# edlanglois/relearn

Measured on AMD Instinct MI355X. Metric: env-steps/sec (whole node), 64k-env CartPole TRPO, higher is better.
Workload: dtype f32; 1 GPU; CartPole(VisibleStepLimit 500) MLP-TRPO, 65536 envs total, T=128, policy 5-128-2, critic 5-128-1, CG 10, <=15 backtracks, 80 Adam critic steps per period; n_envs_total=65536, n_envs_per_gpu=65536, horizon=128, hidden=128, critic_steps=80, update_chains=policy and critic chains side by side on two streams, pipeline=none, parallelism=env-sharded x1 + no collective (one rank)

## Files before the change

include/relearn_hip.h:

```cpp
#ifndef RELEARN_HIP_H
#define RELEARN_HIP_H

#include <stddef.h>
#include <stdint.h>

#ifdef __cplusplus
extern "C" {
#endif

#define RL_ABI_VERSION 6

typedef enum {
  RL_OK = 0,
  RL_ERR_INVALID_ARGUMENT = 1,
  RL_ERR_HIP = 2,
  RL_ERR_NO_DEVICE = 3,
  RL_ERR_BUILD_AGENT = 4,
  RL_ERR_BUILD_ENV = 5,
  RL_ERR_BUFFER_FULL = 6,
  RL_ERR_PACKING = 7,
  RL_ERR_COMM = 8,
  RL_ERR_OPT_NAN = 9,
  RL_ERR_UNSUPPORTED = 10
} rl_status;
// ... 75 lines not shown
  uint64_t episodes_per_trial;
} rl_meta_bandit_config;
int32_t rl_meta_bandit_config_default(rl_meta_bandit_config *meta);
int32_t rl_env_create_meta_bandit(rl_engine *engine, const rl_env_config *cfg, const rl_meta_bandit_config *meta,
                                  rl_env **out);
int32_t rl_env_create_meta_bandit_wide(rl_engine *engine, const rl_env_config *cfg, const rl_meta_bandit_config *meta,
                                       rl_env **out);
int32_t rl_env_destroy(rl_env *env);
int32_t rl_env_dims(const rl_env *env, uint32_t *obs_dim, uint32_t *n_actions);
int32_t rl_env_reset(rl_env *env);
int32_t rl_env_observe(rl_env *env, float *obs_out);
int32_t rl_env_step(rl_env *env, const uint8_t *actions, float *reward_out, uint8_t *flag_out, float *obs_out,
                    float *term_obs_out);
int32_t rl_env_upload_actions(rl_env *env, const uint8_t *actions);
int32_t rl_env_step_resident(rl_env *env);
int32_t rl_env_get_state(rl_env *env, double *state4, int32_t *nv_pos, uint64_t *steps_remaining,
                         uint64_t *reset_count);
int32_t rl_env_set_state(rl_env *env, const double *state4, const int32_t *nv_pos, const uint64_t *steps_remaining,
                         const uint64_t *reset_count);

int32_t rl_debug_stream_words(rl_engine *engine, uint64_t seed, uint64_t stream, uint64_t first_word, uint32_t n_words,
                              uint32_t *words_out);
int32_t rl_debug_device_memory(uint64_t *live_bytes, uint64_t *live_allocations);

int32_t rl_mlp_create(rl_engine *engine, uint32_t in_dim, uint32_t hidden, uint32_t out_dim, rl_mlp **out);
typedef enum {
  RL_ACT_IDENTITY = 0,
  RL_ACT_RELU = 1,
  RL_ACT_SIGMOID = 2,
  RL_ACT_TANH = 3
} rl_activation;
int32_t rl_mlp_create_layers(rl_engine *engine, uint32_t in_dim, const uint32_t *hidden_sizes, uint32_t n_hidden,
                             uint32_t out_dim, int32_t activation, int32_t output_activation, rl_mlp **out);
int32_t rl_mlp_create_config(rl_engine *engine, uint32_t in_dim, const uint32_t *hidden_sizes, uint32_t n_hidden,
                             uint32_t out_dim, int32_t activation, int32_t output_activation, int32_t bias, rl_mlp **out);
int32_t rl_mlp_destroy(rl_mlp *mlp);
int32_t rl_mlp_num_params(const rl_mlp *mlp, uint64_t *n);
int32_t rl_mlp_init(rl_mlp *mlp, uint64_t seed);
typedef enum { RL_INIT_ZEROS = 0, RL_INIT_CONSTANT = 1, RL_INIT_UNIFORM = 2, RL_INIT_NORMAL = 3, RL_INIT_ORTHOGONAL = 4 } rl_init_kind;
typedef enum { RL_SCALE_CONSTANT = 0, RL_SCALE_FAN_IN = 1, RL_SCALE_FAN_OUT = 2, RL_SCALE_FAN_AVG = 3 } rl_variance_scale;
typedef struct {
  int32_t kind;
  int32_t scale;
  double value;
} rl_initializer;
int32_t rl_mlp_init_with(rl_mlp *mlp, uint64_t seed, const rl_initializer *kernel_init, const rl_initializer *bias_init);
// ... 264 lines not shown
```

relearn_amd/__init__.py:

```python
import atexit
import ctypes as C
import math
import os
import subprocess
import sys
import weakref

import numpy as np

_HERE = os.path.dirname(os.path.abspath(__file__))
LIB_PATH = os.environ.get("RELEARN_LIB", os.path.join(_HERE, "librelearn_hip.so"))
CSRC = os.path.join(_HERE, "csrc")

OK = 0
ERR_INVALID_ARGUMENT, ERR_HIP, ERR_NO_DEVICE, ERR_BUILD_AGENT, ERR_BUILD_ENV = 1, 2, 3, 4, 5
ERR_BUFFER_FULL, ERR_PACKING, ERR_COMM, ERR_OPT_NAN, ERR_UNSUPPORTED = 6, 7, 8, 9, 10
SUCC_CONTINUE, SUCC_TERMINATE, SUCC_INTERRUPT = 0, 1, 2
OPT_OK, OPT_LOSS_NOT_IMPROVING, OPT_CONSTRAINT_VIOLATED, OPT_NAN_LOSS, OPT_NAN_CONSTRAINT = range(5)
ENV_CARTPOLE, ENV_CHAIN, ENV_MEMORY, ENV_BANDIT, ENV_META_BANDIT = 0, 1, 2, 3, 4
BANDITS_UNIFORM_BERNOULLI, BANDITS_ONE_HOT, BANDITS_ROUND_ROBIN = 0, 1, 2
BANDIT_DISTRIBUTIONS = {"uniform_bernoulli": BANDITS_UNIFORM_BERNOULLI, "one_hot": BANDITS_ONE_HOT,
                        "round_robin": BANDITS_ROUND_ROBIN}
LIMIT_NONE, LIMIT_LATENT, LIMIT_VISIBLE = 0, 1, 2
BANDIT_AGENT_RANDOM, BANDIT_AGENT_TABULAR_Q, BANDIT_AGENT_UCB1 = 0, 1, 2
BANDIT_AGENT_THOMPSON = 4
BANDIT_AGENT_KINDS = {"random": BANDIT_AGENT_RANDOM, "tabular_q": BANDIT_AGENT_TABULAR_Q, "ucb1": BANDIT_AGENT_UCB1,
                      "thompson": BANDIT_AGENT_THOMPSON}
(BANDIT_STATE_ACTOR_POS, BANDIT_STATE_COUNTS, BANDIT_STATE_VALUES, BANDIT_STATE_VISITS,
 BANDIT_STATE_LN_TABLE, BANDIT_STATE_LOW_COUNTS, BANDIT_STATE_HIGH_COUNTS) = range(7)
(TRAJ_OBS, TRAJ_ACTION, TRAJ_REWARD, TRAJ_FLAG, TRAJ_TERM_OBS, TRAJ_VALUES, TRAJ_ADVANTAGES,
 TRAJ_RETURNS, TRAJ_TARGETS) = range(9)
VALUE_TARGET_REWARD_TO_GO, VALUE_TARGET_ONE_STEP_TD = 0, 1
OPTIMIZER_ADAM, OPTIMIZER_ADAMW, OPTIMIZER_SGD, OPTIMIZER_RMSPROP = 0, 1, 2, 3
KERNEL_CLASSES = ["env_step", "rollout", "values", "gae", "policy_pass", "backward", "reduce", "small",
                  "critic_fwd", "allreduce", "critic_fused", "policy_fused", "policy_fvp"]

ABI_SYMBOLS = [
    "rl_abi_version", "rl_debug_stream_words", "rl_debug_device_memory", "rl_device_count", "rl_engine_create", "rl_engine_destroy", "rl_engine_sync",
    "rl_last_error", "rl_engine_info", "rl_engine_set_kernel_variant", "rl_timer_begin", "rl_timer_end", "rl_profile_enable", "rl_profile_read",
    "rl_comm_available", "rl_comm_library_paths", "rl_comm_unique_id", "rl_comm_init", "rl_comm_destroy", "rl_comm_init_host",
    "rl_comm_ipc_handle", "rl_comm_init_ipc", "rl_comm_selftest",
    "rl_cartpole_params_default", "rl_env_create", "rl_env_create_bandit", "rl_meta_bandit_config_default", "rl_env_create_meta_bandit", "rl_env_create_meta_bandit_wide", "rl_env_destroy", "rl_env_dims", "rl_env_reset",
    "rl_env_observe", "rl_env_step", "rl_env_upload_actions", "rl_env_step_resident", "rl_env_get_state",
    "rl_env_set_state",
    "rl_mlp_create", "rl_mlp_create_layers", "rl_mlp_create_config", "rl_mlp_destroy", "rl_mlp_num_params", "rl_mlp_init", "rl_mlp_init_with", "rl_params_get", "rl_params_set",
    "rl_mlp_forward", "rl_gru_mlp_create", "rl_lstm_mlp_create", "rl_rnn_mlp_create", "rl_rnn_mlp_create_config", "rl_rnn_linear_create", "rl_rnn_chain_config_default", "rl_rnn_chain_create", "rl_rnn_chain_create_wide", "rl_rnn_mlp_init_with", "rl_seq_forward",
    "rl_traj_create", "rl_traj_destroy", "rl_traj_field_bytes", "rl_traj_read", "rl_traj_write",
    "rl_rollout", "rl_gae",
    "rl_trpo_config_default", "rl_trpo_update", "rl_policy_gradient", "rl_policy_fvp", "rl_policy_loss_kl",
    "rl_adam_config_default", "rl_adam_create", "rl_adam_destroy", "rl_adam_step_host",
    "rl_optimizer_config_default", "rl_optimizer_create", "rl_optimizer_step_host", "rl_optimizer_state_read",
    "rl_critic_update", "rl_critic_gradient", "rl_values_opt_config_default", "rl_values_opt_update",
    "rl_actor_critic_update", "rl_actor_critic_update_begin", "rl_actor_critic_update_finish", "rl_engine_set_serial_update",
    "rl_ppo_config_default", "rl_ppo_update", "rl_reinforce_update", "rl_reward_to_go",
    "rl_actor_to_cbor", "rl_module_from_cbor", "rl_tensor_def_to_cbor", "rl_tensor_def_from_cbor",
    "rl_indexed_type_space_to_cbor",
    "rl_dqn_config_default", "rl_dqn_create", "rl_dqn_create_recurrent", "rl_dqn_create_finite", "rl_dqn_destroy", "rl_dqn_exploration_rate",
    "rl_dqn_min_update_size", "rl_dqn_collect", "rl_dqn_update", "rl_dqn_replay_field_bytes", "rl_dqn_replay_read",
    "rl_dqn_minibatch_sample", "rl_dqn_minibatch_read", "rl_dqn_minibatch_gradient", "rl_dqn_agent_rng_pos",
    "rl_chain_tabular_q_train", "rl_chain_tabular_q_eval",
    "rl_summary_create", "rl_summary_destroy", "rl_summary_push", "rl_summary_push_dqn", "rl_summary_read",
# ... 670 lines not shown

    def close(self):
        if self.h:
            lib().rl_traj_destroy(self.h)
            self.h = C.c_void_p()

    def shape(self, field):
        n, T, D = self.n, self.T, self.D
        return {TRAJ_OBS: (D, T + 1, n), TRAJ_ACTION: (T, n), TRAJ_REWARD: (T, n), TRAJ_FLAG: (T, n),
                TRAJ_TERM_OBS: (D, T, n), TRAJ_VALUES: (T + 1, n), TRAJ_ADVANTAGES: (T, n),
                TRAJ_RETURNS: (T, n), TRAJ_TARGETS: (T, n)}[field]

    def read(self, field):
        out = np.zeros(self.shape(field), dtype=_TRAJ_DTYPES[field])
        _check(lib().rl_traj_read(self.h, C.c_int32(field), out.ctypes.data_as(C.c_void_p),
                                  C.c_uint64(out.nbytes)), self.eng.h)
        return out

    def write(self, field, arr):
        arr, ap = _ptr(arr, _TRAJ_DTYPES[field])
        assert arr.shape == self.shape(field), (arr.shape, self.shape(field))
        _check(lib().rl_traj_write(self.h, C.c_int32(field), ap, C.c_uint64(arr.nbytes)), self.eng.h)

    def read_all(self):
        return dict(obs=self.read(TRAJ_OBS), action=self.read(TRAJ_ACTION), reward=self.read(TRAJ_REWARD),
                    flag=self.read(TRAJ_FLAG), term_obs=self.read(TRAJ_TERM_OBS))

    def write_all(self, traj):
        self.write(TRAJ_OBS, traj["obs"])
        self.write(TRAJ_ACTION, traj["action"])
        self.write(TRAJ_REWARD, traj["reward"])
        self.write(TRAJ_FLAG, traj["flag"])
        self.write(TRAJ_TERM_OBS, traj["term_obs"])


def rollout(env, policy, traj):
    _check(lib().rl_rollout(env.h, policy.h, traj.h), env.eng.h)


def gae(traj, critic, gamma, lam):
    _check(lib().rl_gae(traj.h, critic.h, C.c_float(gamma), C.c_float(lam)), traj.eng.h)


def trpo_config_default():
    c = TrpoConfig()
    _check(lib().rl_trpo_config_default(C.byref(c)))
# ... 513 lines not shown
```

relearn_amd/csrc/abi.hip:

```cpp
#include <dlfcn.h>

#include <atomic>
#include <condition_variable>
#include <map>
#include <mutex>

#include "abi_internal.hpp"
#include "env_lanes.hpp"

thread_local std::string g_last_error_no_engine;

static std::atomic<uint64_t> g_device_bytes{0}, g_device_allocations{0};

void *rl_device_alloc(uint64_t bytes) {
  void *p = nullptr;
  RL_HIP_CHECK(hipMalloc(&p, bytes));
  g_device_bytes += bytes;
  g_device_allocations += 1;
  return p;
}

void rl_device_free(void *p, uint64_t bytes) {
  (void)hipFree(p);
  g_device_bytes -= bytes;
// ... 298 lines not shown
    if (compute_units) *compute_units = e->prop.multiProcessorCount;
  });
}

int32_t rl_timer_begin(rl_engine *e) {
  return guarded(e, [&] {
    RL_REQUIRE(e, "engine is NULL");
    RL_HIP_CHECK(hipEventRecord(e->ev_begin, e->stream));
  });
}

int32_t rl_timer_end(rl_engine *e, float *elapsed_ms) {
  return guarded(e, [&] {
    RL_REQUIRE(e && elapsed_ms, "NULL argument");
    RL_HIP_CHECK(hipEventRecord(e->ev_end, e->stream));
    RL_HIP_CHECK(hipEventSynchronize(e->ev_end));
    RL_HIP_CHECK(hipEventElapsedTime(elapsed_ms, e->ev_begin, e->ev_end));
  });
}

int32_t rl_engine_set_kernel_variant(rl_engine *e, int32_t variant) {
  return guarded(e, [&] {
    RL_REQUIRE(e, "engine is NULL");
    RL_REQUIRE(variant == 0 || variant == 1, "kernel variant must be 0 (best) or 1 (v1 reference kernels)");
    e->kernel_variant = variant;
  });
}

int32_t rl_engine_set_serial_update(rl_engine *e, int32_t serial) {
  return guarded(e, [&] {
    RL_REQUIRE(e, "engine is NULL");
    e->serial_update = serial != 0;
  });
}

int32_t rl_profile_enable(rl_engine *e, int32_t on) {
  return guarded(e, [&] {
    RL_REQUIRE(e, "engine is NULL");
    sync(e);
    prof_drain(e);
    e->profiling = on != 0;
  });
}

int32_t rl_profile_read(rl_engine *e, double *total_ms_out, uint64_t *launches_out, int32_t reset) {
  return guarded(e, [&] {
    RL_REQUIRE(e, "engine is NULL");
// ... 448 lines not shown

int32_t rl_debug_stream_words(rl_engine *engine, uint64_t seed, uint64_t stream, uint64_t first_word, uint32_t n_words,
                              uint32_t *words_out) {
  return guarded(engine, [&] {
    RL_REQUIRE(engine && words_out, "NULL argument");
    RL_REQUIRE(n_words > 0 && n_words <= (1u << 20), "n_words must be in [1, 2^20]");
    AgentKey key;
    rl_seed_from_u64(seed, key.w);
    DevMem tmp;
    uint32_t *d = tmp.alloc<uint32_t>(n_words);
    hipLaunchKernelGGL(k_debug_stream_words, dim3((n_words + 255) / 256), dim3(256), 0, engine->stream, key, stream,
                       first_word, n_words, d);
    RL_HIP_CHECK(hipGetLastError());
    d2h(engine, words_out, d, (size_t)n_words * sizeof(uint32_t));
  });
}

int32_t rl_debug_device_memory(uint64_t *live_bytes, uint64_t *live_allocations) {
  if (live_bytes) *live_bytes = g_device_bytes.load();
  if (live_allocations) *live_allocations = g_device_allocations.load();
  return RL_OK;
}

int32_t rl_env_upload_actions(rl_env *env, const uint8_t *actions) {
  return guarded(env ? env->eng : nullptr, [&] {
    RL_REQUIRE(env && actions, "NULL argument");
    check_actions(env, actions);
    h2d(env->eng, env->d_actions, actions, env->cfg.n_lanes);
  });
}

int32_t rl_env_step_resident(rl_env *env) {
  return guarded(env ? env->eng : nullptr, [&] {
    RL_REQUIRE(env, "env is NULL");
    launch_env_step(env);
    env->t_global += 1;
  });
}

int32_t rl_env_step(rl_env *env, const uint8_t *actions, float *reward_out, uint8_t *flag_out, float *obs_out,
                    float *term_obs_out) {
  return guarded(env ? env->eng : nullptr, [&] {
    RL_REQUIRE(env && actions, "NULL argument");
    check_actions(env, actions);
    rl_engine *e = env->eng;
    size_t n = env->cfg.n_lanes;
// ... 805 lines not shown
```

relearn_amd/csrc/abi_dqn.hip:

```cpp
#include "abi_internal.hpp"

extern "C" {

int32_t rl_dqn_config_default(rl_dqn_config *c) {
  return guarded(nullptr, [&] {
    RL_REQUIRE(c, "cfg is NULL");
    std::memset(c, 0, sizeof(*c));
    c->target = RL_DQN_TARGET_REWARD_TO_GO;
    c->exploration_kind = RL_SCHEDULE_LINEAR_ANNEALED;
    c->exploration_start = 1.0;
    c->exploration_end = 0.1;
    c->exploration_period = 10000000;
    c->minibatch_steps = 100000;
    c->opt_steps_per_update = 50;
    c->buffer_capacity = 0;
    c->episode_capacity = 0;
    c->update_kind = RL_COLLECT_FIRST_REST;
    c->update_first = 1000000;
    c->update_rest = 100000;
    c->discount_factor = 0.99f;
  });
}

static double dqn_exploration_rate(const rl_dqn *q, bool training) {
// ... 415 lines not shown
                         q->d_ep_off + o, q->d_counts + k, mb->d.obs, 0, mb->d.action, mb->d.adv, 0,
                         q->cfg.discount_factor, mb->d.flag);
    q->mem.ensure(q->d_q_next, (uint64_t)q->A * q->max_steps_mb);
    launch_gen_forward(mb, q->qnet, mb->d.obs + c.n_steps, (size_t)2 * c.n_steps, c.n_steps, q->d_q_next);
    launch_dqn_td_targets(q->eng, mb->d.adv, mb->d.flag, q->d_q_next, c.n_steps, q->A, q->cfg.discount_factor);
    return;
  }
  launch_dqn_build_minibatch(q->eng, q->rp, c.n_eps, q->d_ep_lane + o, q->d_ep_start + o, q->d_ep_len + o,
                             q->d_ep_off + o, mb->d.obs, (size_t)2 * c.n_steps, mb->d.action, mb->d.adv,
                             q->cfg.discount_factor, td ? 1 : 0, q->qnet);
}

static void dqn_sample_minibatch(rl_dqn *q, int sequential) {
  std::vector<DqnCountsDev> counts;
  std::vector<uint64_t> totals;
  dqn_draw_minibatches(q, sequential, 1, counts, totals);
  dqn_build_minibatch(q, 0, counts[0], totals[0]);
}

static void dqn_gradient(rl_dqn *q, rl_adam *step_opt = nullptr, int loss_slot = -1) {
  if (q->recurrent) return rdqn_gradient(q, step_opt, loss_slot);
  rl_traj *mb = q->mb;
  bool fused = false;
  if (q->eng->kernel_variant == 0)
    fused = q->td_in_kernel ? launch_dqn_step_bf16(mb, q->qnet, q->last_total_steps, q->cfg.discount_factor)
                            : launch_dqn_step_pair(mb, q->qnet, q->last_total_steps);
  PassRequest pass(RUN_DQN);
  pass.B_total = q->last_total_steps;
  pass.reduce = false;
  const SlabRows rows = fused ? SlabRows{mb->nbV2, mb->nbV2} : run_pass(q->qnet, mb, pass);
  if (step_opt && !q->eng->has_collective()) {
    launch_reduce_opt(mb, step_opt, rows.A, rows.B, loss_slot, q->last_total_steps);
    return;
  }
  const uint32_t P = (uint32_t)q->qnet->P;
  launch_reduce(mb, P, true, true, rows.A, rows.B);
  rl_allreduce_sum_f32(q->eng, mb->vec, P + 4);
  if (step_opt) launch_opt_step(mb, step_opt, loss_slot, q->last_total_steps);
}

static void rdqn_update(rl_dqn *q, rl_dqn_update_stats *stats, float *losses_out) {
  rl_engine *e = q->eng;
  if (e->n_ranks > 1)
    throw RlError(RL_ERR_UNSUPPORTED, "rl_dqn_update: an agent of rl_dqn_create_recurrent updates on one rank");
  q->global_steps = q->steps_per_lane * (uint64_t)q->rp.N;
  const uint64_t K = q->cfg.opt_steps_per_update;
  std::vector<DqnCountsDev> counts;
// ... 33 lines not shown
  }
  std::vector<float> h(K ? K : 1, 0.0f);
  if (K) d2h(e, h.data(), q->seq->losses, K * sizeof(float));
  if (losses_out && K) std::memcpy(losses_out, h.data(), K * sizeof(float));
  if (stats) {
    stats->opt_steps = K;
    stats->loss_first = K ? (double)h[0] : 0.0;
    stats->loss_last = K ? (double)h[K - 1] : 0.0;
    stats->global_steps = q->global_steps;
    stats->last_minibatch_steps = q->last_n_steps;
    stats->last_minibatch_episodes = q->last_n_eps;
  }
}

int32_t rl_dqn_update(rl_dqn *q, rl_dqn_update_stats *stats, float *losses_out) {
  return guarded(q ? q->eng : nullptr, [&] {
    RL_REQUIRE(q, "NULL argument");
    if (q->recurrent) return rdqn_update(q, stats, losses_out);
    rl_engine *e = q->eng;
    q->global_steps = q->steps_per_lane * (uint64_t)q->rp.N * (uint64_t)e->n_ranks;
    uint64_t K = q->cfg.opt_steps_per_update;
    const uint64_t D = q->rp.D, cap = q->max_steps_mb;
    const bool td = q->cfg.target == RL_DQN_TARGET_ONE_STEP_TD;
    const bool fused_shape = e->kernel_variant == 0 && fused_5_128_fits(q->mb, q->qnet, 2, false);
    const bool td_fused = td && fused_shape;
    const bool all_at_once = K > 1 && (!td || td_fused) && K * cap * (8 * D + 6) <= (8ull << 30);
    if (all_at_once) {
      q->mem.ensure(q->all_obs, K * D * 2 * cap);
      q->mem.ensure(q->all_target, K * cap);
      q->mem.ensure(q->all_action, K * cap);
      if (td) q->mem.ensure(q->all_flag, K * cap);
    }
    const bool pipelined = all_at_once && e->n_ranks == 1 && !e->profiling;
    std::vector<DqnCountsDev> counts;
    std::vector<uint64_t> totals;
    std::vector<uint32_t> chunk_end;
    if (pipelined) {
      for (uint64_t first = 0, size = 2; first < K; first += size, size *= 2) chunk_end.push_back((uint32_t)(first + size < K ? first + size : K));
      if (!q->draw_stream) RL_HIP_CHECK(hipStreamCreateWithFlags(&q->draw_stream, hipStreamNonBlocking));
      if (!q->main_event) RL_HIP_CHECK(hipEventCreateWithFlags(&q->main_event, hipEventDisableTiming));
      if (!q->h_counts) q->h_counts = q->mem.alloc_host<DqnCountsDev>(K, false);
      while (q->draw_events.size() < chunk_end.size()) {
        hipEvent_t ev;
        RL_HIP_CHECK(hipEventCreateWithFlags(&ev, hipEventDisableTiming));
        q->draw_events.push_back(ev);
      }
      RL_HIP_CHECK(hipEventRecord(q->main_event, e->stream));
// ... 216 lines not shown
```

relearn_amd/csrc/abi_update.hip:

```cpp
#include "abi_internal.hpp"

enum FusedLauncher { FUSED_NONE, FUSED_POLICY ,
                     FUSED_CRITIC  };
struct PassRow {
  bool backward, sums;
  FusedLauncher fused;
};
static const PassRow PASS_TABLE[RUN_KINDS] = {
     {true, true, FUSED_POLICY},
     {false, true, FUSED_POLICY},
     {true, false, FUSED_POLICY},
     {true, true, FUSED_NONE},
     {true, true, FUSED_POLICY},
     {true, true, FUSED_CRITIC},
};
static_assert(RUN_INIT == 0 && RUN_EVAL == 1 && RUN_JVP == 2 && RUN_DQN == 3 && RUN_PPO == 4 && RUN_CRITIC == 5 &&
                  RUN_KINDS == 6,
              "PASS_TABLE rows are in the order of PassKind");

static void seq_gradient_to_flat_order(const rl_mlp *mod, rl_traj *traj) {
  if (mod->exec == nullptr) return;
  launch_seq_unpad(mod, traj->vec, mod->x_tmp);
  RL_HIP_CHECK(hipMemcpyAsync(traj->vec, mod->x_tmp, mod->P * sizeof(float), hipMemcpyDeviceToDevice, traj->eng->stream));
}
// ... 18 lines not shown
    seq_ensure(traj, sc.x, true);
    if (req.kind == RUN_JVP) {
      const float *tangent = req.tangent;
      if (mod->exec != nullptr) {
        launch_seq_pad(mod, mod->x_tan, req.tangent);
        tangent = mod->x_tan;
      }
      launch_gru_tangent(traj, sc.x, tangent, Bt, req.skip);
    } else {
      launch_gru_seq_forward(traj, sc.x, traj->seq.out, nullptr, row.backward ? seq_record(traj, sc.x) : nullptr,
                             req.skip);
      if (critic) launch_seq_critic_dvalues(traj, Bt);
      else launch_seq_policy_dlogits(traj, req.kind, Bt, req.clip_lo, req.clip_hi, req.skip, sc.x->out_dim);
    }
    if (grad) {
      launch_gru_backward(traj, sc.x, req.skip);
      seq_gradient_to_flat_order(mod, traj);
    }
    if (row.sums) launch_reduce(traj, P, false, true, 0, traj->nbB);
    allreduce();
    return SlabRows{0, traj->nbB};
  }
  bool fused = false;
  if (traj->eng->kernel_variant == 0) {
    if (row.fused == FUSED_POLICY)
      fused = launch_policy_v2(traj, mod, req.kind, req.tangent, Bt, req.skip, req.clip_lo, req.clip_hi, req.keep);
    else if (row.fused == FUSED_CRITIC)
      fused = launch_critic_step_v2(traj, mod, Bt);
  }
  if (!fused) {
    if (critic) launch_critic_fwd(traj, mod, Bt);
    else launch_policy_pass(traj, mod, req.kind, req.tangent, Bt, req.skip, req.clip_lo, req.clip_hi);
    if (row.backward) launch_mlp_backward(traj, mod, req.skip);
  }
  const SlabRows rows = fused ? SlabRows{traj->last_rows, traj->last_rows} : SlabRows{traj->nbA, traj->nbB};
  if (req.reduce) {
    launch_reduce(traj, P, row.backward, row.sums, rows.A, rows.B);
    allreduce();
  }
  return rows;
}

extern "C" {

int32_t rl_trpo_config_default(rl_trpo_config *c) {
  return guarded(nullptr, [&] {
    RL_REQUIRE(c, "cfg is NULL");
// ... 677 lines not shown
```

relearn_amd/csrc/kernels_general.hip:

```cpp
#include <mutex>
#include <set>

#include "abi_internal.hpp"
#include "env_lanes.hpp"
#include "policy_terms.hpp"

namespace {

constexpr int GT = 64;

static inline uint32_t cdiv_g(size_t a, size_t b) { return (uint32_t)((a + b - 1) / b); }

__device__ __forceinline__ float act_apply(int act, float x) {
  if (act == RL_ACT_RELU) return x > 0.0f ? x : 0.0f;
  if (act == RL_ACT_SIGMOID) return rl_sigmoidf(x);
  if (act == RL_ACT_TANH) return rl_tanhf(x);
  return x;
}
__device__ __forceinline__ float act_slope(int act, float y) {
  if (act == RL_ACT_RELU) return y > 0.0f ? 1.0f : 0.0f;
  if (act == RL_ACT_SIGMOID) return y * (1.0f - y);
  if (act == RL_ACT_TANH) return 1.0f - y * y;
  return 1.0f;
}
// ... 711 lines not shown
  GenDev &g = t->gen;
  const size_t plane = (size_t)(T + 1) * n;
  if (!g.no_interrupt) g.no_interrupt = t->mem.alloc<int32_t>(1);
  RL_HIP_CHECK(hipMemsetAsync(g.no_interrupt, 1, sizeof(int32_t), t->eng->stream));
  hipLaunchKernelGGL(k_gen_any_interrupt, dim3(256), dim3(256), 0, t->eng->stream, t->d, g.no_interrupt);
  auto fwd = [&](const float *x, size_t xs, uint64_t rows, float *out, const int32_t *skip) {
    if (!launch_gen_chain_rows(t->eng, critic, x, xs, rows, out, (size_t)rows, skip))
      gen_forward_impl(t, critic, x, xs, rows, out, nullptr, nullptr, skip);
  };
  fwd(t->d.term_obs, (size_t)B, B, g.z, g.no_interrupt);
  fwd(t->d.obs + (size_t)T * n, plane, n, g.z + B, nullptr);
  hipLaunchKernelGGL(k_gen_successor_values, dim3(cdiv_g(B, 256)), dim3(256), 0, t->eng->stream, t->d, g.z, g.z + B,
                     q.succ);
  fwd(t->d.obs, plane, B, q.out, nullptr);
  return g.z + B;
}

void launch_gen_rollout(rl_env *env, const rl_mlp *policy, rl_traj *t) {
  rl_engine *e = env->eng;
  const uint32_t n = t->d.n, T = t->d.T;
  gen_ensure(t, policy, n, false, false);
  GenDev &g = t->gen;
  ChainNet net;
  if (env->kind == RL_ENV_CARTPOLE && policy->out_dim == 2 && e->kernel_variant == 0 && chain_net(policy, &net)) {
    const size_t lds = ((size_t)2 * net.wmax * GT + 16 * GT) * sizeof(float);
    if (env->D == 5) {
      chain_lds_attr(e, reinterpret_cast<const void *>(&k_gen_rollout_cartpole<5>), lds);
      hipLaunchKernelGGL(k_gen_rollout_cartpole<5>, dim3(cdiv_g(n, GT)), dim3(ROLL_WAVES * 64), lds, e->stream, env->dev, env->st, t->d,
                         net, env->t_global);
    } else {
      chain_lds_attr(e, reinterpret_cast<const void *>(&k_gen_rollout_cartpole<4>), lds);
      hipLaunchKernelGGL(k_gen_rollout_cartpole<4>, dim3(cdiv_g(n, GT)), dim3(ROLL_WAVES * 64), lds, e->stream, env->dev, env->st, t->d,
                         net, env->t_global);
    }
    RL_HIP_CHECK(hipGetLastError());
    env->t_global += T;
    return;
  }
  launch_rollout_stepwise(env, t, g.z, [&](uint32_t) {
    gen_forward_impl(t, policy, env->d_obs, (size_t)n, n, g.z, nullptr, nullptr, nullptr);
  });
}

void launch_rollout_stepwise(rl_env *env, rl_traj *t, const float *z, const std::function<void(uint32_t)> &forward) {
  rl_engine *e = env->eng;
  const uint32_t n = t->d.n, T = t->d.T;
  const dim3 grid(cdiv_g(n, 256)), blk(256);
// ... 55 lines not shown
```

relearn_amd/csrc/kernels_rollout.hip:

```cpp
#include <type_traits>

#include "bf16_tile.hpp"
#include "device_fns.hpp"
#include "env_lanes.hpp"
#include "kernels.hpp"

template <class Env>
__global__ void k_env_reset(CartPoleDev c, EnvStateDev st, uint32_t n) {
  uint32_t i = blockIdx.x * blockDim.x + threadIdx.x;
  if (i >= n) return;
  typename Env::State s;
  Env::load(st, i, s);
  Env::reset(c, s, c.lane_offset + i);
  Env::store(st, i, s);
}

template <class Env, int D>
__global__ void k_env_observe(CartPoleDev c, EnvStateDev st, uint32_t n, float *__restrict__ obs) {
  uint32_t i = blockIdx.x * blockDim.x + threadIdx.x;
  if (i >= n) return;
  typename Env::State s;
  Env::load(st, i, s);
  float f[D];
  Env::template features<D>(c, s, f);
#pragma unroll
  for (int d = 0; d < D; ++d) obs[(size_t)d * n + i] = f[d];
}

// ... 50 lines not shown
    float z[2], lp[2];
    mlp_forward_group_lds<D, G>(pk, H, g, f, z);
    log_softmax_lane<2>(z, lp);
    int a = categorical_sample_lane<2>(lp, u);
    const TrajSink sink{tr, (size_t)t * n + il, writer};
    float reward;
    const int succ = Env::step(c, s, a, lane, t_global + t, reward);
    sink.record(a, reward, succ);
    if (succ == RL_SUCC_INTERRUPT) {
      Env::features<D>(c, s, f);
      sink.successor(f);
    }
    if (succ != RL_SUCC_CONTINUE) Env::reset(c, s, lane);
  }
  float f[D];
  Env::features<D>(c, s, f);
  if (writer) {
#pragma unroll
    for (int d = 0; d < D; ++d) tr.obs[d * plane + (size_t)T * n + il] = f[d];
    Env::store(st, il, s);
  }
}

template <int D, int A, bool RANGE = false>
__global__ void __launch_bounds__(256) k_mlp_forward_rows(const float *__restrict__ params, int H,
                                                          const float *__restrict__ in, size_t in_plane,
                                                          size_t rows, float *__restrict__ out, size_t out_plane,
                                                          uint32_t *__restrict__ range = nullptr) {
  size_t r = (size_t)blockIdx.x * blockDim.x + threadIdx.x;
  if (!RANGE && r >= rows) return;
  const bool live = r < rows;
  float x[D], z[A];
#pragma unroll
  for (int d = 0; d < D; ++d) x[d] = live ? in[d * in_plane + r] : 0.0f;
  if (RANGE) {
    uint32_t lo = 0x7F7FFFFFu, hi = 0u;
#pragma unroll
    for (int d = 0; d < D; ++d) {
      const uint32_t a = __builtin_bit_cast(uint32_t, x[d]) & 0x7FFFFFFFu;
      hi = a > hi ? a : hi;
      lo = a != 0u && a < lo ? a : lo;
    }
#pragma unroll
    for (int m = 32; m > 0; m >>= 1) {
      const uint32_t ol = (uint32_t)__shfl_xor((int)lo, m, 64), oh = (uint32_t)__shfl_xor((int)hi, m, 64);
      lo = ol < lo ? ol : lo;
      hi = oh > hi ? oh : hi;
    }
    if ((threadIdx.x & 63) == 0) bt::range_fold(range, blockIdx.x * 4 + (threadIdx.x >> 6), lo, hi);
    if (!live) return;
  }
  mlp_forward_lane<D, A>(params, H, x, z);
#pragma unroll
  for (int a = 0; a < A; ++a) out[a * out_plane + r] = z[a];
}

template <int D>
__device__ __forceinline__ float critic_value_of(const float *__restrict__ critic, int H, const float *__restrict__ x0,
                                              size_t stride) {
  float x[D], z[1];
#pragma unroll
  for (int d = 0; d < D; ++d) x[d] = x0[(size_t)d * stride];
  mlp_forward_lane<D, 1>(critic, H, x, z);
  return z[0];
}

template <int D>
__global__ void __launch_bounds__(256) k_gae_scan(TrajDev tr, const float *__restrict__ critic, int H, float gamma,
                                                  float lambda, int rtg_only) {
  const uint32_t n = tr.n, T = tr.T;
  uint32_t i = blockIdx.x * blockDim.x + threadIdx.x;
  if (i >= n) return;
  const float disc = lambda * gamma;
  float adv_next = 0.0f, rtg_next = 0.0f;
  if (rtg_only) {
    for (uint32_t t = T; t-- > 0;) {
      size_t o = (size_t)t * n + i;
// ... 240 lines not shown
#define ENV_STEP(FF)                                                                                                    \
  hipLaunchKernelGGL((k_env_step<Env, D, FF>), dim3(cdiv(n, 256)), dim3(256), 0, env->eng->stream, env->dev, env->st, n, \
                     env->d_actions, env->d_reward, env->d_flag, env->d_obs, env->d_term_obs, env->t_global)
    if constexpr (std::is_same_v<Env, CartPoleOps>) {
      if (n >= (1u << 20)) {
        ENV_STEP(true);
        return;
      }
    }
    ENV_STEP(false);
#undef ENV_STEP
  });
}

template <int D, int G>
static void launch_rollout_g(rl_env *env, const rl_mlp *policy, rl_traj *traj) {
  constexpr int BLOCK = 64;
  const uint32_t n = (uint32_t)env->cfg.n_lanes;
  hipLaunchKernelGGL((k_rollout_cartpole<D, BLOCK, G>), dim3(cdiv((size_t)n * G, BLOCK)), dim3(BLOCK), 0,
                     env->eng->stream, env->dev, env->st, traj->d, policy->d_params, (int)policy->hidden, env->t_global);
  traj->range_reset = true;
}

void launch_rollout(rl_env *env, const rl_mlp *policy, rl_traj *traj) {
  ProfScope ps(env->eng, RL_K_ROLLOUT);
  const uint64_t simds = 4ull * (uint64_t)env->eng->prop.multiProcessorCount, n = env->cfg.n_lanes;
  int G = 1;
  while (G < 16 && n * (uint64_t)(2 * G) <= (2 * G >= 8 ? 1 : 2) * simds * 64) G *= 2;
#define ROLL(DD)                                                   \
  switch (G) {                                                     \
    case 16: launch_rollout_g<DD, 16>(env, policy, traj); break;   \
    case 8: launch_rollout_g<DD, 8>(env, policy, traj); break;     \
    case 4: launch_rollout_g<DD, 4>(env, policy, traj); break;     \
    case 2: launch_rollout_g<DD, 2>(env, policy, traj); break;     \
    default: launch_rollout_g<DD, 1>(env, policy, traj); break;    \
  }
  if (env->D == 5) {
    ROLL(5)
  } else {
    ROLL(4)
  }
#undef ROLL
}

void launch_values(rl_traj *traj, const rl_mlp *critic) {
  ProfScope ps(traj->eng, RL_K_VALUES);
  size_t rows = (size_t)(traj->d.T + 1) * traj->d.n;
  if (traj->d.D == 5 && traj->range_reset && !traj->range_valid && !traj->range_fixed) {
    hipLaunchKernelGGL((k_mlp_forward_rows<5, 1, true>), dim3(cdiv(rows, 256)), dim3(256), 0, traj->eng->stream,
                       critic->d_params, (int)critic->hidden, traj->d.obs, rows, rows, traj->d.values, rows, traj->d.range);
    traj->range_valid = true;
    traj->range_reset = false;
  } else if (traj->d.D == 5)
    hipLaunchKernelGGL((k_mlp_forward_rows<5, 1>), dim3(cdiv(rows, 256)), dim3(256), 0, traj->eng->stream,
                       critic->d_params, (int)critic->hidden, traj->d.obs, rows, rows, traj->d.values, rows, (uint32_t *)nullptr);
  else
    hipLaunchKernelGGL((k_mlp_forward_rows<4, 1>), dim3(cdiv(rows, 256)), dim3(256), 0, traj->eng->stream,
                       critic->d_params, (int)critic->hidden, traj->d.obs, rows, rows, traj->d.values, rows, (uint32_t *)nullptr);
}

void launch_gae(rl_traj *traj, const rl_mlp *critic, float gamma, float lambda) {
  ProfScope ps(traj->eng, RL_K_GAE);
  uint32_t n = traj->d.n;
  traj->rtg_scan_valid = true;
  traj->rtg_gamma = gamma;
  if (traj->d.D == 5)
    hipLaunchKernelGGL(k_gae_scan<5>, dim3(cdiv(n, 64)), dim3(64), 0, traj->eng->stream, traj->d,
                       critic ? critic->d_params : (const float *)nullptr, critic ? (int)critic->hidden : 0, gamma, lambda,
                       critic ? 0 : 1);
  else
    hipLaunchKernelGGL(k_gae_scan<4>, dim3(cdiv(n, 64)), dim3(64), 0, traj->eng->stream, traj->d,
                       critic ? critic->d_params : (const float *)nullptr, critic ? (int)critic->hidden : 0, gamma, lambda,
                       critic ? 0 : 1);
}

void launch_value_targets(rl_traj *traj, const rl_mlp *critic, float gamma) {
  ProfScope ps(traj->eng, RL_K_GAE);
  if (critic == nullptr) {
    hipLaunchKernelGGL(k_value_targets_rtg, dim3(cdiv(traj->d.n, 64)), dim3(64), 0, traj->eng->stream, traj->d, gamma);
    return;
  }
  const size_t B = (size_t)traj->d.T * traj->d.n;
  if (traj->d.D == 5)
    hipLaunchKernelGGL(k_value_targets_td<5>, dim3(cdiv(B, 256)), dim3(256), 0, traj->eng->stream, traj->d,
                       critic->d_params, (int)critic->hidden, gamma);
  else
    hipLaunchKernelGGL(k_value_targets_td<4>, dim3(cdiv(B, 256)), dim3(256), 0, traj->eng->stream, traj->d,
                       critic->d_params, (int)critic->hidden, gamma);
}

void launch_mlp_forward_host_rows(rl_mlp *mlp, const float *d_in_soa, size_t rows, float *d_out_soa) {
  ProfScope ps(mlp->eng, RL_K_VALUES);
  dim3 g(cdiv(rows, 256)), b(256);
  hipStream_t s = mlp->eng->stream;
  int H = (int)mlp->hidden;
#define FWD(DD, AA)                                                                                              \
  hipLaunchKernelGGL((k_mlp_forward_rows<DD, AA, false>), g, b, 0, s, mlp->d_params, H, d_in_soa, rows, rows, d_out_soa, \
                     rows)
  if (mlp->in_dim == 5 && mlp->out_dim == 2) FWD(5, 2);
  else if (mlp->in_dim == 5 && mlp->out_dim == 1) FWD(5, 1);
  else if (mlp->in_dim == 4 && mlp->out_dim == 2) FWD(4, 2);
  else if (mlp->in_dim == 4 && mlp->out_dim == 1) FWD(4, 1);
  else throw RlError(RL_ERR_UNSUPPORTED, "mlp forward: unsupported (in_dim, out_dim)");
#undef FWD
}
```

Measured before the change: 518.9 million env-steps/s.

## Run rollout and critic value MLP forward on MFMA matrix units

Adds a tiled MLP forward for hidden size 128 that computes layer 1 with 32x32x2 f32 MFMA instructions and layer 2 with packed FMAs over a shared-memory weight image. It is used in the CartPole rollout kernel when there are at least 16k lanes, and in the critic value and host-row forward passes. Two new kernel variants force the tile path, and a debug entry point exposes the observation range words. The aim is to replace per-lane scalar MLP evaluation with matrix-unit work and reuse of shared weights. In exchange it uses 64-thread blocks with half-wave duplication, and the changed summation order may alter numerics.

Measured after the change: 519.0 million env-steps/s, median of 3. About the same (+0.0%).

```diff
diff --git a/include/relearn_hip.h b/include/relearn_hip.h
--- a/include/relearn_hip.h
+++ b/include/relearn_hip.h
@@ -121,6 +121,7 @@
 int32_t rl_debug_stream_words(rl_engine *engine, uint64_t seed, uint64_t stream, uint64_t first_word, uint32_t n_words,
                               uint32_t *words_out);
 int32_t rl_debug_device_memory(uint64_t *live_bytes, uint64_t *live_allocations);
+int32_t rl_debug_obs_range(rl_traj *traj, uint32_t *words_out , int32_t *valid_out);
 
 int32_t rl_mlp_create(rl_engine *engine, uint32_t in_dim, uint32_t hidden, uint32_t out_dim, rl_mlp **out);
 typedef enum {
diff --git a/relearn_amd/__init__.py b/relearn_amd/__init__.py
--- a/relearn_amd/__init__.py
+++ b/relearn_amd/__init__.py
@@ -36,7 +36,7 @@
                   "critic_fwd", "allreduce", "critic_fused", "policy_fused", "policy_fvp"]
 
 ABI_SYMBOLS = [
-    "rl_abi_version", "rl_debug_stream_words", "rl_debug_device_memory", "rl_device_count", "rl_engine_create", "rl_engine_destroy", "rl_engine_sync",
+    "rl_abi_version", "rl_debug_stream_words", "rl_debug_device_memory", "rl_debug_obs_range", "rl_device_count", "rl_engine_create", "rl_engine_destroy", "rl_engine_sync",
     "rl_last_error", "rl_engine_info", "rl_engine_set_kernel_variant", "rl_timer_begin", "rl_timer_end", "rl_profile_enable", "rl_profile_read",
     "rl_comm_available", "rl_comm_library_paths", "rl_comm_unique_id", "rl_comm_init", "rl_comm_destroy", "rl_comm_init_host",
     "rl_comm_ipc_handle", "rl_comm_init_ipc", "rl_comm_selftest",
@@ -753,6 +753,11 @@
         assert arr.shape == self.shape(field), (arr.shape, self.shape(field))
         _check(lib().rl_traj_write(self.h, C.c_int32(field), ap, C.c_uint64(arr.nbytes)), self.eng.h)
 
+    def debug_obs_range(self):
+        words, valid = np.zeros(128, dtype=np.uint32), C.c_int32()
+        _check(lib().rl_debug_obs_range(self.h, words.ctypes.data_as(C.c_void_p), C.byref(valid)), self.eng.h)
+        return words[:64], words[64:], bool(valid.value)
+
     def read_all(self):
         return dict(obs=self.read(TRAJ_OBS), action=self.read(TRAJ_ACTION), reward=self.read(TRAJ_REWARD),
                     flag=self.read(TRAJ_FLAG), term_obs=self.read(TRAJ_TERM_OBS))
diff --git a/relearn_amd/csrc/abi.hip b/relearn_amd/csrc/abi.hip
--- a/relearn_amd/csrc/abi.hip
+++ b/relearn_amd/csrc/abi.hip
@@ -344,7 +344,8 @@
 int32_t rl_engine_set_kernel_variant(rl_engine *e, int32_t variant) {
   return guarded(e, [&] {
     RL_REQUIRE(e, "engine is NULL");
-    RL_REQUIRE(variant == 0 || variant == 1, "kernel variant must be 0 (best) or 1 (v1 reference kernels)");
+    RL_REQUIRE(variant >= 0 && variant <= 3,
+               "kernel variant must be 0 (best), 1 (v1 reference kernels), 2 or 3 (0, matrix-unit rollout at every lane count)");
     e->kernel_variant = variant;
   });
 }
@@ -839,6 +840,16 @@
   return RL_OK;
 }
 
+int32_t rl_debug_obs_range(rl_traj *t, uint32_t *words_out, int32_t *valid_out) {
+  return guarded(t ? t->eng : nullptr, [&] {
+    RL_REQUIRE(t && words_out && valid_out, "NULL argument");
+    std::vector<uint32_t> raw(RL_RANGE_WORDS);
+    d2h(t->eng, raw.data(), t->d.range, raw.size() * sizeof(uint32_t));
+    for (int s = 0; s < 2 * 64; ++s) words_out[s] = raw[(size_t)s * 32];
+    *valid_out = t->range_valid ? 1 : 0;
+  });
+}
+
 int32_t rl_env_upload_actions(rl_env *env, const uint8_t *actions) {
   return guarded(env ? env->eng : nullptr, [&] {
     RL_REQUIRE(env && actions, "NULL argument");
diff --git a/relearn_amd/csrc/abi_dqn.hip b/relearn_amd/csrc/abi_dqn.hip
--- a/relearn_amd/csrc/abi_dqn.hip
+++ b/relearn_amd/csrc/abi_dqn.hip
@@ -461,7 +461,7 @@
   if (q->recurrent) return rdqn_gradient(q, step_opt, loss_slot);
   rl_traj *mb = q->mb;
   bool fused = false;
-  if (q->eng->kernel_variant == 0)
+  if (q->eng->kernel_variant != 1)
     fused = q->td_in_kernel ? launch_dqn_step_bf16(mb, q->qnet, q->last_total_steps, q->cfg.discount_factor)
                             : launch_dqn_step_pair(mb, q->qnet, q->last_total_steps);
   PassRequest pass(RUN_DQN);
@@ -541,7 +541,7 @@
     uint64_t K = q->cfg.opt_steps_per_update;
     const uint64_t D = q->rp.D, cap = q->max_steps_mb;
     const bool td = q->cfg.target == RL_DQN_TARGET_ONE_STEP_TD;
-    const bool fused_shape = e->kernel_variant == 0 && fused_5_128_fits(q->mb, q->qnet, 2, false);
+    const bool fused_shape = e->kernel_variant != 1 && fused_5_128_fits(q->mb, q->qnet, 2, false);
     const bool td_fused = td && fused_shape;
     const bool all_at_once = K > 1 && (!td || td_fused) && K * cap * (8 * D + 6) <= (8ull << 30);
     if (all_at_once) {
diff --git a/relearn_amd/csrc/abi_update.hip b/relearn_amd/csrc/abi_update.hip
--- a/relearn_amd/csrc/abi_update.hip
+++ b/relearn_amd/csrc/abi_update.hip
@@ -64,7 +64,7 @@
     return SlabRows{0, traj->nbB};
   }
   bool fused = false;
-  if (traj->eng->kernel_variant == 0) {
+  if (traj->eng->kernel_variant != 1) {
     if (row.fused == FUSED_POLICY)
       fused = launch_policy_v2(traj, mod, req.kind, req.tangent, Bt, req.skip, req.clip_lo, req.clip_hi, req.keep);
     else if (row.fused == FUSED_CRITIC)
diff --git a/relearn_amd/csrc/kernels_general.hip b/relearn_amd/csrc/kernels_general.hip
--- a/relearn_amd/csrc/kernels_general.hip
+++ b/relearn_amd/csrc/kernels_general.hip
@@ -757,7 +757,7 @@
   gen_ensure(t, policy, n, false, false);
   GenDev &g = t->gen;
   ChainNet net;
-  if (env->kind == RL_ENV_CARTPOLE && policy->out_dim == 2 && e->kernel_variant == 0 && chain_net(policy, &net)) {
+  if (env->kind == RL_ENV_CARTPOLE && policy->out_dim == 2 && e->kernel_variant != 1 && chain_net(policy, &net)) {
     const size_t lds = ((size_t)2 * net.wmax * GT + 16 * GT) * sizeof(float);
     if (env->D == 5) {
       chain_lds_attr(e, reinterpret_cast<const void *>(&k_gen_rollout_cartpole<5>), lds);
diff --git a/relearn_amd/csrc/kernels_rollout.hip b/relearn_amd/csrc/kernels_rollout.hip
--- a/relearn_amd/csrc/kernels_rollout.hip
+++ b/relearn_amd/csrc/kernels_rollout.hip
@@ -4,6 +4,7 @@
 #include "device_fns.hpp"
 #include "env_lanes.hpp"
 #include "kernels.hpp"
+#include "mlp_tile.hpp"
 
 template <class Env>
 __global__ void k_env_reset(CartPoleDev c, EnvStateDev st, uint32_t n) {
@@ -100,6 +101,71 @@
   }
 }
 
+template <int D, int ROWS>
+__global__ void __launch_bounds__(64, 2) k_rollout_cartpole_tile(CartPoleDev c, EnvStateDev st, TrajDev tr,
+                                                                 const float *__restrict__ policy, uint64_t t_global) {
+  using Env = CartPoleOps;
+  constexpr int BLOCK = 64;
+  __shared__ uint32_t actor_words[16 * BLOCK];
+  __shared__ __attribute__((aligned(16))) float w2[mt::W2_FLOATS<2>];
+  const uint32_t n = tr.n, T = tr.T;
+  mt::Layer1<D> l1;
+  l1.load(policy, (int)threadIdx.x);
+  mt::pack_w2<D, 2>(w2, policy, (int)threadIdx.x, BLOCK);
+  if (blockIdx.x == 0) bt::range_reset(tr.range, (int)threadIdx.x, BLOCK);
+  __syncthreads();
+  const int hf = (int)threadIdx.x >> 5;
+  const uint32_t i = ROWS == 64 ? blockIdx.x * 64u + threadIdx.x : blockIdx.x * 32u + (threadIdx.x & 31u);
+  const bool live = i < n;
+  const uint32_t il = live ? i : n - 1;
+  const bool writer = live && (ROWS == 64 || hf == 0);
+  const uint64_t lane = c.lane_offset + il;
+  Env::State s;
+  Env::load(st, il, s);
+  const size_t plane = (size_t)(T + 1) * n;
+  LaneActorRng<BLOCK> rng{&actor_words[threadIdx.x], c.key_actor, lane, t_global, ~0ull};
+  for (uint32_t t = 0; t < T; ++t) {
+    float f[D];
+    Env::features<D>(c, s, f);
+    if (writer) {
+#pragma unroll
+      for (int d = 0; d < D; ++d) tr.obs[d * plane + (size_t)t * n + il] = f[d];
+    }
+    rng.pos = t_global + t;
+    const float u = rl_u32_to_unit_f32(rng.next_u32());
+    float z[2], lp[2];
+    if (ROWS == 64) {
+      float xt[2][D], z0[2], z1[2];
+#pragma unroll
+      for (int d = 0; d < D; ++d) bt::both_halves(f[d], xt[0][d], xt[1][d]);
+      mt::forward<D, 2>(l1, w2, hf, xt[0], z0);
+      mt::forward<D, 2>(l1, w2, hf, xt[1], z1);
+      z[0] = hf ? z1[0] : z0[0];
+      z[1] = hf ? z1[1] : z0[1];
+    } else {
+      mt::forward<D, 2>(l1, w2, hf, f, z);
+    }
+    log_softmax_lane<2>(z, lp);
+    int a = categorical_sample_lane<2>(lp, u);
+    const TrajSink sink{tr, (size_t)t * n + il, writer};
+    float reward;
+    const int succ = Env::step(c, s, a, lane, t_global + t, reward);
+    sink.record(a, reward, succ);
+    if (succ == RL_SUCC_INTERRUPT) {
+      Env::features<D>(c, s, f);
+      sink.successor(f);
+    }
+    if (succ != RL_SUCC_CONTINUE) Env::reset(c, s, lane);
+  }
+  float f[D];
+  Env::features<D>(c, s, f);
+  if (writer) {
+#pragma unroll
+    for (int d = 0; d < D; ++d) tr.obs[d * plane + (size_t)T * n + il] = f[d];
+    Env::store(st, il, s);
+  }
+}
+
 template <int D, int A, bool RANGE = false>
 __global__ void __launch_bounds__(256) k_mlp_forward_rows(const float *__restrict__ params, int H,
                                                           const float *__restrict__ in, size_t in_plane,
@@ -131,6 +197,56 @@
   mlp_forward_lane<D, A>(params, H, x, z);
 #pragma unroll
   for (int a = 0; a < A; ++a) out[a * out_plane + r] = z[a];
+}
+
+template <int D, int A, bool RANGE>
+__global__ void __launch_bounds__(256, 2) k_mlp_forward_rows_tile(const float *__restrict__ params,
+                                                               const float *__restrict__ in, size_t in_plane, size_t rows,
+                                                               float *__restrict__ out, size_t out_plane,
+                                                               uint32_t *__restrict__ range) {
+  __shared__ __attribute__((aligned(16))) float w2[mt::W2_FLOATS<A>];
+  mt::Layer1<D> l1;
+  l1.load(params, (int)threadIdx.x & 63);
+  mt::pack_w2<D, A>(w2, params, (int)threadIdx.x, 256);
+  __syncthreads();
+  const int ln = (int)threadIdx.x & 63, hf = ln >> 5;
+  const size_t r0 = (size_t)blockIdx.x * 256 + (threadIdx.x & ~63u);
+  const size_t r = r0 + ln;
+  const bool live = r < rows;
+  float x[D];
+#pragma unroll
+  for (int d = 0; d < D; ++d) x[d] = live ? in[d * in_plane + r] : 0.0f;
+  if (RANGE) {
+    uint32_t lo = 0x7F7FFFFFu, hi = 0u;
+#pragma unroll
+    for (int d = 0; d < D; ++d) {
+      const uint32_t a = __builtin_bit_cast(uint32_t, x[d]) & 0x7FFFFFFFu;
+      hi = a > hi ? a : hi;
+      lo = a != 0u && a < lo ? a : lo;
+    }
+#pragma unroll
+    for (int m = 32; m > 0; m >>= 1) {
+      const uint32_t ol = (uint32_t)__shfl_xor((int)lo, m, 64), oh = (uint32_t)__shfl_xor((int)hi, m, 64);
+      lo = ol < lo ? ol : lo;
+      hi = oh > hi ? oh : hi;
+    }
+    if (ln == 0) bt::range_fold(range, blockIdx.x * 4 + (threadIdx.x >> 6), lo, hi);
+  }
+  if (r0 >= rows) return;
+  float xt[2][D];
+#pragma unroll
+  for (int d = 0; d < D; ++d) bt::both_halves(x[d], xt[0][d], xt[1][d]);
+#pragma unroll
+  for (int tile = 0; tile < 2; ++tile) {
+    if (r0 + 32 * tile >= rows) break;
+    float z[A];
+    mt::forward<D, A>(l1, w2, hf, xt[tile], z);
+    const size_t row = r0 + 32 * tile + (ln & 31);
+    if (hf == 0 && row < rows) {
+#pragma unroll
+      for (int a = 0; a < A; ++a) out[a * out_plane + row] = z[a];
+    }
+  }
 }
 
 template <int D>
@@ -417,9 +533,28 @@
   traj->range_reset = true;
 }
 
+constexpr uint64_t TILE_ROLLOUT_MIN_LANES = 16384;
+static bool rollout_takes_tile(const rl_engine *e, const rl_mlp *policy, uint64_t n) {
+  if (policy->hidden != mt::H || e->kernel_variant == 1) return false;
+  return e->kernel_variant >= 2 || n >= TILE_ROLLOUT_MIN_LANES;
+}
+
 void launch_rollout(rl_env *env, const rl_mlp *policy, rl_traj *traj) {
   ProfScope ps(env->eng, RL_K_ROLLOUT);
   const uint64_t simds = 4ull * (uint64_t)env->eng->prop.multiProcessorCount, n = env->cfg.n_lanes;
+  if (rollout_takes_tile(env->eng, policy, n)) {
+    const bool rows64 = env->eng->kernel_variant == 3;
+#define ROLL_TILE(DD, RR)                                                                                               \
+  hipLaunchKernelGGL((k_rollout_cartpole_tile<DD, RR>), dim3(cdiv(n, RR)), dim3(64), 0, env->eng->stream, env->dev, env->st, \
+                     traj->d, policy->d_params, env->t_global)
+    if (env->D == 5 && rows64) ROLL_TILE(5, 64);
+    else if (env->D == 5) ROLL_TILE(5, 32);
+    else if (rows64) ROLL_TILE(4, 64);
+    else ROLL_TILE(4, 32);
+#undef ROLL_TILE
+    traj->range_reset = true;
+    return;
+  }
   int G = 1;
   while (G < 16 && n * (uint64_t)(2 * G) <= (2 * G >= 8 ? 1 : 2) * simds * 64) G *= 2;
 #define ROLL(DD)                                                   \
@@ -441,17 +576,31 @@
 void launch_values(rl_traj *traj, const rl_mlp *critic) {
   ProfScope ps(traj->eng, RL_K_VALUES);
   size_t rows = (size_t)(traj->d.T + 1) * traj->d.n;
+  const bool tile = critic->hidden == mt::H && traj->eng->kernel_variant != 1;
+#define VALUES_TILE(DD, RR)                                                                                             \
+  hipLaunchKernelGGL((k_mlp_forward_rows_tile<DD, 1, RR>), dim3(cdiv(rows, 256)), dim3(256), 0, traj->eng->stream,      \
+                     critic->d_params, traj->d.obs, rows, rows, traj->d.values, rows, traj->d.range)
   if (traj->d.D == 5 && traj->range_reset && !traj->range_valid && !traj->range_fixed) {
+    if (tile) {
+      VALUES_TILE(5, true);
+      traj->range_valid = true;
+      traj->range_reset = false;
+      return;
+    }
     hipLaunchKernelGGL((k_mlp_forward_rows<5, 1, true>), dim3(cdiv(rows, 256)), dim3(256), 0, traj->eng->stream,
                        critic->d_params, (int)critic->hidden, traj->d.obs, rows, rows, traj->d.values, rows, traj->d.range);
     traj->range_valid = true;
     traj->range_reset = false;
+  } else if (tile) {
+    if (traj->d.D == 5) VALUES_TILE(5, false);
+    else VALUES_TILE(4, false);
   } else if (traj->d.D == 5)
     hipLaunchKernelGGL((k_mlp_forward_rows<5, 1>), dim3(cdiv(rows, 256)), dim3(256), 0, traj->eng->stream,
                        critic->d_params, (int)critic->hidden, traj->d.obs, rows, rows, traj->d.values, rows, (uint32_t *)nullptr);
   else
     hipLaunchKernelGGL((k_mlp_forward_rows<4, 1>), dim3(cdiv(rows, 256)), dim3(256), 0, traj->eng->stream,
                        critic->d_params, (int)critic->hidden, traj->d.obs, rows, rows, traj->d.values, rows, (uint32_t *)nullptr);
+#undef VALUES_TILE
 }
 
 void launch_gae(rl_traj *traj, const rl_mlp *critic, float gamma, float lambda) {
@@ -489,7 +638,19 @@
   dim3 g(cdiv(rows, 256)), b(256);
   hipStream_t s = mlp->eng->stream;
   int H = (int)mlp->hidden;
-#define FWD(DD, AA)                                                                                              \
+  if (mlp->hidden == mt::H && mlp->eng->kernel_variant != 1 && (mlp->in_dim == 4 || mlp->in_dim == 5) &&
+      (mlp->out_dim == 1 || mlp->out_dim == 2)) {
+#define FWD_TILE(DD, AA)                                                                                             \
+  hipLaunchKernelGGL((k_mlp_forward_rows_tile<DD, AA, false>), g, b, 0, s, mlp->d_params, d_in_soa, rows, rows, d_out_soa, \
+                     rows, (uint32_t *)nullptr)
+    if (mlp->in_dim == 5 && mlp->out_dim == 2) FWD_TILE(5, 2);
+    else if (mlp->in_dim == 5) FWD_TILE(5, 1);
+    else if (mlp->out_dim == 2) FWD_TILE(4, 2);
+    else FWD_TILE(4, 1);
+#undef FWD_TILE
+    return;
+  }
+#define FWD(DD, AA)                                                                                           \
   hipLaunchKernelGGL((k_mlp_forward_rows<DD, AA, false>), g, b, 0, s, mlp->d_params, H, d_in_soa, rows, rows, d_out_soa, \
                      rows)
   if (mlp->in_dim == 5 && mlp->out_dim == 2) FWD(5, 2);
diff --git a/relearn_amd/csrc/mlp_tile.hpp b/relearn_amd/csrc/mlp_tile.hpp
--- /dev/null
+++ b/relearn_amd/csrc/mlp_tile.hpp
@@ -0,0 +1,95 @@
+#pragma once
+
+#include "bf16_tile.hpp"
+#include "device_fns.hpp"
+
+namespace mt {
+using bt::f32x16;
+constexpr int H = 128, NT = 4, KS = 3;
+
+__host__ __device__ constexpr int unit_of(int t, int r, int hf) { return 32 * t + 8 * (r >> 2) + 4 * hf + (r & 3); }
+template <int A>
+constexpr int W2_FLOATS = 2 * NT * 16 * A + 4;
+
+template <int D>
+struct Layer1 {
+  float w[NT][KS];
+  __device__ __forceinline__ void load(const float *__restrict__ params, int lane) {
+    static_assert(D == 4 || D == 5, "six k slots: the bias and four or five inputs");
+    const int m = lane & 31, hf = lane >> 5;
+#pragma unroll
+    for (int t = 0; t < NT; ++t)
+#pragma unroll
+      for (int s = 0; s < KS; ++s) {
+        const int j = 32 * t + m, k = 2 * s + hf;
+        w[t][s] = k == 0 ? params[H * D + j] : k <= D ? params[j * D + k - 1] : 0.0f;
+      }
+  }
+};
+
+template <int D, int A>
+__device__ __forceinline__ void pack_w2(float *__restrict__ img, const float *__restrict__ params, int tid, int nthreads) {
+  const float *__restrict__ W2 = params + H * D + H;
+  for (int q = tid; q < 2 * NT * 16 * A; q += nthreads) {
+    const int a = q % A, r = (q / A) & 15, t = (q / (16 * A)) & 3, hf = q / (NT * 16 * A);
+    img[q] = W2[a * H + unit_of(t, r, hf)];
+  }
+  if (tid < A) img[2 * NT * 16 * A + tid] = W2[A * H + tid];
+}
+
+__device__ __forceinline__ float relu1(float c) {
+  const int b = __builtin_bit_cast(int, c);
+  return __builtin_bit_cast(float, b > 0 ? b : 0);
+}
+
+template <int D, int A>
+__device__ __forceinline__ void forward(const Layer1<D> &l1, const float *__restrict__ img, int hf, const float (&x)[D],
+                                        float (&z)[A]) {
+  static_assert(A == 1 || A == 2, "one or two outputs");
+  float xb[KS];
+  xb[0] = hf ? x[0] : 1.0f;
+  xb[1] = hf ? x[2] : x[1];
+  xb[2] = hf ? (D == 5 ? x[D - 1] : 0.0f) : x[3];
+  float c[A][8];
+  bt::f32x2 cp[8];
+#pragma unroll
+  for (int q = 0; q < 8; ++q) {
+    cp[q] = bt::f32x2{0.0f, 0.0f};
+#pragma unroll
+    for (int a = 0; a < A; ++a) c[a][q] = 0.0f;
+  }
+  const float *__restrict__ w2 = img + hf * (NT * 16 * A);
+#pragma unroll
+  for (int t = 0; t < NT; ++t) {
+    f32x16 acc = {0, 0, 0, 0, 0, 0, 0, 0, 0, 0, 0, 0, 0, 0, 0, 0};
+#pragma unroll
+    for (int s = 0; s < KS; ++s) acc = __builtin_amdgcn_mfma_f32_32x32x2f32(l1.w[t][s], xb[s], acc, 0, 0, 0);
+    float u[16 * A];
+#pragma unroll
+    for (int v = 0; v < 4 * A; ++v) {
+      const float4 q4 = *reinterpret_cast<const float4 *>(w2 + t * 16 * A + 4 * v);
+      u[4 * v] = q4.x, u[4 * v + 1] = q4.y, u[4 * v + 2] = q4.z, u[4 * v + 3] = q4.w;
+    }
+#pragma unroll
+    for (int r = 0; r < 16; ++r) {
+      const float h = relu1(acc[r]);
+      const int q = (r & 3) + 4 * ((r >> 2) & 1);
+      if constexpr (A == 2) cp[q] = __builtin_elementwise_fma(bt::f32x2{h, h}, bt::f32x2{u[2 * r], u[2 * r + 1]}, cp[q]);
+      else c[0][q] = __builtin_fmaf(h, u[r], c[0][q]);
+    }
+  }
+  if constexpr (A == 2) {
+#pragma unroll
+    for (int q = 0; q < 8; ++q) c[0][q] = cp[q].x, c[1][q] = cp[q].y;
+  }
+#pragma unroll
+  for (int a = 0; a < A; ++a) {
+    const float p0 = (c[a][0] + c[a][1]) + (c[a][2] + c[a][3]);
+    const float p1 = (c[a][4] + c[a][5]) + (c[a][6] + c[a][7]);
+    float p0l, p0h, p1l, p1h;
+    bt::both_halves(p0, p0l, p0h);
+    bt::both_halves(p1, p1l, p1h);
+    z[a] = ((p0l + p0h) + (p1l + p1h)) + img[2 * NT * 16 * A + a];
+  }
+}
+}
```
